# ma921/BASQ

Measured on NVIDIA B200. Metric: candidate points recombined/sec (N->n, d=10), higher is better.
Workload: dtype f32 kernel evaluation (fp16 hi/lo split distance contraction, 3 products), f64 accumulation/projection/Caratheodory

## Files before the change

basq_b200/_lib.py:

```python
from __future__ import annotations

import ctypes as C
import os

_HERE = os.path.dirname(os.path.abspath(__file__))
LIB_PATH = os.environ.get("BASQ_B200_LIB") or os.path.join(_HERE, "libbasq_b200.so")

BASQ_MAX_DIM = 32
OK, ERR_INVALID, ERR_CUDA, ERR_NUMERIC, ERR_UNSUPPORTED = range(5)
RBF, MATERN15, MATERN25 = 0, 1, 2
PLAIN, PRED_COV, WSABI_L, WSABI_M, MMLT_G = 0, 1, 2, 3, 4
F32, F64 = 0, 1
PHASES = ("prepare", "set_sum", "projection", "caratheodory", "apply", "nystrom", "gp_predict", "other")


class BasqError(RuntimeError):
    def __init__(self, code, msg):
        super().__init__(f"basq_b200 error {code}: {msg}")
        self.code = code


class KernelDesc(C.Structure):
    _fields_ = [
        ("family", C.c_int32), ("mode", C.c_int32), ("dtype", C.c_int32), ("d", C.c_int32),
# ... 33 lines not shown
        "basq_nystrom_basis_sharded": (I, [P, KD, P, L, I, P, I, I, I, P, P, P, P, P]),
        "basq_nystrom_basis": (I, [P, KD, P, L, I, P, I, P, P]),
        "basq_features": (I, [P, KD, P, L, P, L, P, I, P]),
        "basq_car": (I, [P, P, I, I, I, P, C.POINTER(I)]),
        "basq_recombine": (I, [P, KD, P, L, P, L, P, I, P, P, P, C.POINTER(I)]),
        "basq_recombine_objective": (I, [P, KD, P, L, P, L, P, I, P, P, P, P, C.POINTER(I)]),
        "basq_car_objective": (I, [P, P, I, I, I, P]),
        "basq_session_set_objective": (I, [P, P]),
        "basq_recombine_host": (I, [P, KD, P, L, P, L, P, I, P, I, P, P, P, C.POINTER(I)]),
        "basq_session_create": (I, [P, KD, P, L, L, L, P, L, P, I, P, C.POINTER(P)]),
        "basq_session_destroy": (None, [P]),
        "basq_session_count": (I, [P, C.POINTER(L)]),
        "basq_session_partial": (I, [P, L, L, P]),
        "basq_session_apply": (I, [P, L, L, P, C.POINTER(L)]),
        "basq_session_result": (I, [P, P, P, I, C.POINTER(I)]),
        "basq_session_cell_factor": (I, [P, L, L, C.POINTER(I)]),
        "basq_session_pass_begin": (I, [P, L, L, I]),
        "basq_session_level": (I, [P, I, I, P, P, P, P]),
        "basq_session_landmarks": (I, [P, C.POINTER(I)]),
        "basq_session_level_fold": (I, [P, I, I, P, P, L]),
        "basq_session_level_project": (I, [P, I, I, P, P, P, P, L, I, I, P]),
        "basq_session_apply_cells": (I, [P, L, L, I, P, C.POINTER(L)]),
        "basq_sample_mvn": (I, [P, C.c_uint64, L, L, I, I, P, P, P]),
        "basq_standard_normals": (I, [P, C.c_uint64, L, L, I, P]),
        "basq_ctx_set_seed": (I, [P, C.c_uint64]),
        "basq_ctx_memory": (I, [P, C.POINTER(C.c_uint64), C.POINTER(C.c_uint64), C.POINTER(L)]),
        "basq_ctx_allow_f32_eval": (I, [P, I, C.POINTER(L)]),
        "basq_mvn_logpdf": (I, [P, P, L, I, I, P, P, P]),
        "basq_candidate_weights": (I, [P, I, D, I, P, P, L, I, P]),
        "basq_cleanse_weights": (I, [P, P, L, D]),
        "basq_sir_resample": (I, [P, P, L, L, C.c_uint64, P, C.POINTER(L)]),
        "basq_dgemm": (I, [P, I, I, I, I, I, D, P, I, P, I, D, P, I]),
        "basq_tgemm": (I, [P, I, I, I, P, I, P, I, P, I]),
    }
    for name, (res, args) in sig.items():
        fn = getattr(lib, name)
        fn.restype = res
        fn.argtypes = args
    return lib, tuple(sig)


lib, SYMBOLS = _load()


def check(code):
    if code != OK:
        raise BasqError(code, lib.basq_last_error().decode("utf-8", "replace"))


class Context:

    def __init__(self, device_index: int, stream_ptr: int = 0):
        h = C.c_void_p()
        check(lib.basq_ctx_create(int(device_index), C.c_void_p(stream_ptr or None), C.byref(h)))
        self.handle = h
        self.device_index = device_index
        self.stream_ptr = stream_ptr

    def __del__(self):
        h, self.handle = getattr(self, "handle", None), None
        if h and lib is not None:
            lib.basq_ctx_destroy(h)

    @property
    def launches(self) -> int:
        return int(lib.basq_ctx_launch_count(self.handle))
# ... 55 lines not shown
```

basq_b200/csrc/api.cu:

```cuda
#include <math.h>
#include <string.h>
#include <stdlib.h>

#include <algorithm>
#include <memory>
#include <new>

#include "common.cuh"
#include "tgemm.cuh"

namespace basq {
const char* last_error_cstr();

namespace {

__global__ void scale_columns_kernel(double* __restrict__ U, int rows, int cols, int64_t ld,
                                     const double* __restrict__ s) {
  const int64_t t = (int64_t)blockIdx.x * blockDim.x + threadIdx.x;
  if (t >= (int64_t)rows * cols) return;
  const int r = (int)(t / cols), c = (int)(t % cols);
  U[(int64_t)r * ld + c] *= s[c];
}

__global__ void warp_gram_kernel(double* __restrict__ C, int64_t a, int64_t b, int mode, const double* __restrict__ fx,
                                 const double* __restrict__ fy, double pre_add, double diag_add, int64_t diag_col0) {
  const int64_t t = (int64_t)blockIdx.x * blockDim.x + threadIdx.x;
  if (t >= a * b) return;
  const int64_t i = t / b, j = t % b - diag_col0;
  double c = C[t];
  if (i == j) c += pre_add;
  if (mode == BASQ_WSABI_L) c = fx[i] * c * fy[j + diag_col0];
  else if (mode == BASQ_WSABI_M) c = fx[i] * c * fy[j + diag_col0] + 0.5 * c * c;
  else if (mode == BASQ_MMLT_G) c = fx[i] * fy[j + diag_col0] * expm1(c);
  if (i == j) c += diag_add;
  C[t] = c;
}

__global__ void model_space_kernel(int mode, double offset, int64_t n, double* __restrict__ mean,
                                   double* __restrict__ var, int write_var) {
  const int64_t p = (int64_t)blockIdx.x * blockDim.x + threadIdx.x;
  if (p >= n) return;
// ... 63 lines not shown

int narrow_f64(basq_ctx* ctx, const double* in, int64_t n, float* out) {
  f64_to_f32_kernel<<<(unsigned)ceil_div64(n, 256), 256, 0, ctx->stream>>>(in, n, out);
  ctx->launches++;
  BASQ_CUDA(cudaGetLastError());
  return BASQ_OK;
}

int widen_f32(basq_ctx* ctx, const float* in, int64_t n, double* out) {
  f32_to_f64_kernel<<<(unsigned)ceil_div64(n, 256), 256, 0, ctx->stream>>>(in, n, out);
  ctx->launches++;
  BASQ_CUDA(cudaGetLastError());
  return BASQ_OK;
}

namespace {

int check_finite_host(const double* v, int64_t n, const char* what) {
  for (int64_t i = 0; i < n; ++i)
    BASQ_CHECK(isfinite(v[i]), BASQ_ERR_NUMERIC, "%s contains a non-finite value at %lld", what, (long long)i);
  return BASQ_OK;
}

}
}

using namespace basq;

struct Piece {
  void* p = nullptr;
  template <typename T> T* as() const { return static_cast<T*>(p); }
};

struct basq_session {
  basq_ctx* ctx = nullptr;
  basq_kernel_desc desc;
  KParams kp;
  int M = 0, q = 0, n = 0, S = 0, Mtot = 0;
  int nl = NL_LIN;
  Landmarks lm;
  Landmarks lmobs;
  DevBuf Uprime;
  DevBuf sz;
  DevBuf Az;
  RecPool pool;
  DevBuf G;
  int64_t ldg = 0;
  DevBuf rank;
  int pass_F = 0;
  int64_t pass_R = 0, pass_off = 0;
  const double* obj = nullptr;
  int rows = 0;
  DevBuf cellmass;
  DevBuf cellobj;
  DevBuf Gf;
  DevBuf raw[2];
  int raw_cur = 0;
  DevBuf lnode, lppos, lfpar;
  NlSweep nls;
  DevBuf X64, Z64, Xobs64;
  bool promoted = false;
  double kappa = 0.0;
  int64_t idx_base = 0;
  bool scale_wf = true;
  std::vector<double> omega_host;
  std::vector<int> rank_host;
  DevBuf X32, Z32, Xobs32;
  bool demoted = false;
  const void *origX = nullptr, *origZ = nullptr, *origXobs = nullptr;
};

namespace basq {
namespace {

int session_set_sums(basq_session* s, int64_t off, int S, int64_t p_lo, int64_t p_hi, double* G, int64_t ldg) {
// ... 172 lines not shown
      s->Az.release();
      basq_kernel_desc d64 = *desc;
      d64.dtype = BASQ_F64;
      d64.Xobs = s->Xobs64.p;
      s->promoted = true;
      ctx->promotions++;
      return session_create_impl(ctx, &d64, s->X64.p, N_loc, N_glob, idx_base, s->Z64.p, M, U, q, mu, S_override, s);
    }
  }

  DevBuf sx;
  const bool has_factor = (mode == BASQ_WSABI_L || mode == BASQ_WSABI_M || mode == BASQ_MMLT_G);
  if (has_factor) {
    BASQ_TRY(s->sz.alloc(ctx, sizeof(double) * M));
    BASQ_TRY(warp_factor(ctx, desc, s->kp, s->lmobs.view(), Z, M, s->sz.as<double>()));
    BASQ_TRY(sx.alloc(ctx, sizeof(double) * std::max<int64_t>(N_loc, 1)));
    BASQ_TRY(warp_factor(ctx, desc, s->kp, s->lmobs.view(), X, N_loc, sx.as<double>()));
  }

  BASQ_TRY(s->Uprime.alloc(ctx, sizeof(double) * (size_t)q * s->Mtot));
  BASQ_CUDA(cudaMemcpy2DAsync(s->Uprime.p, sizeof(double) * s->Mtot, U, sizeof(double) * M, sizeof(double) * M, q,
                              cudaMemcpyDeviceToDevice, ctx->stream));
  if (mode == BASQ_WSABI_L) {
    scale_columns_kernel<<<ceil_div((int64_t)q * M, 256), 256, 0, ctx->stream>>>(s->Uprime.as<double>(), q, (int)M,
                                                                                s->Mtot, s->sz.as<double>());
    ctx->launches++;
  }
  if (augment) {
    BASQ_TRY(dgemm(ctx, false, false, q, n_obs, (int)M, -1.0, s->Uprime.as<double>(), s->Mtot, s->Az.as<double>(),
                   n_obs, 0.0, s->Uprime.as<double>() + M, s->Mtot));
    BASQ_CUDA(cudaStreamSynchronize(ctx->stream));
    s->Az.release();
  }

  const double uniform_w = 1.0 / (double)(N_glob > 0 ? N_glob : 1);
  BASQ_TRY(build_records(ctx, s->kp, desc->dtype, X, N_loc, uniform_w, mu, has_factor ? sx.as<double>() : nullptr,
                         !nonlin, &s->pool));

  s->ldg = 0;
  if (nonlin) {
    BASQ_TRY(nl_sweep_prepare(ctx, desc, s->kp, s->Az.as<double>(), (int)M, s->sz.as<double>(), N_loc, &s->nls));
    if (s->nls.use_nls) s->Az.release();
  }
  BASQ_CUDA(cudaStreamSynchronize(ctx->stream));
  return BASQ_OK;
}

int session_reserve_cells(basq_session* s, int cells) {
  if (cells <= s->ldg) return BASQ_OK;
  basq_ctx* ctx = s->ctx;
  BASQ_CUDA(cudaStreamSynchronize(ctx->stream));
  s->G.release();
  s->rank.release();
  s->ldg = cells;
  BASQ_TRY(s->G.alloc(ctx, sizeof(double) * (size_t)s->Mtot * s->ldg));
  BASQ_TRY(s->rank.alloc(ctx, sizeof(int) * (size_t)cells));
  s->cellmass.release();
  s->cellobj.release();
  BASQ_TRY(s->cellmass.alloc(ctx, sizeof(double) * (size_t)cells));
  BASQ_TRY(s->cellobj.alloc(ctx, sizeof(double) * (size_t)cells));
  s->omega_host.resize(cells);
  s->rank_host.resize(cells);
  return BASQ_OK;
}

int session_pass_begin(basq_session* s, int64_t R_glob, int64_t off, int F) {
// ... 83 lines not shown
  const int n = s->n, S = s->S, F = s->pass_F, rows = s->rows;
  BASQ_TRY(session_level_check(s, lvl, K, node_host, ppos_host));
  BASQ_CHECK(row0 >= 0 && nrows >= 0 && row0 + nrows <= s->Mtot, BASQ_ERR_INVALID, "level: bad landmark row range");
  const int stride = S << lvl, cnt = F >> lvl;
  PhaseTimer t(ctx, PH_PROJ);
  {
    unsigned char* slot = nullptr;
    int si = 0;
    BASQ_TRY(stage_take(ctx, (size_t)s->S * 16, &slot, &si));
    int* h_node = reinterpret_cast<int*>(slot);
    int* h_ppos = h_node + S;
    double* h_fpar = reinterpret_cast<double*>(slot + (size_t)S * 8);
    memcpy(h_node, node_host, sizeof(int) * K);
    if (lvl > 0) memcpy(h_ppos, ppos_host, sizeof(int) * K);
    memcpy(h_fpar, fpar_host, sizeof(double) * K);
    BASQ_CUDA(cudaMemcpyAsync(s->lnode.p, h_node, sizeof(int) * K, cudaMemcpyHostToDevice, ctx->stream));
    if (lvl > 0) BASQ_CUDA(cudaMemcpyAsync(s->lppos.p, h_ppos, sizeof(int) * K, cudaMemcpyHostToDevice, ctx->stream));
    BASQ_CUDA(cudaMemcpyAsync(s->lfpar.p, h_fpar, sizeof(double) * K, cudaMemcpyHostToDevice, ctx->stream));
    BASQ_CUDA(cudaEventRecord(ctx->stage_ev[si], ctx->stream));
  }
  BASQ_CUDA(cudaMemsetAsync(A_out, 0, sizeof(double) * (size_t)rows * S, ctx->stream));
  double* raw = s->raw[s->raw_cur].as<double>();
  const double* prev = s->raw[s->raw_cur ^ 1].as<double>();
  fold_cols_kernel<<<(unsigned)ceil_div64(K, 256), 256, 0, ctx->stream>>>(s->cellmass.as<double>(), 0, 1, K,
                                                                          s->lnode.as<int>(), stride, cnt, raw, S);
  ctx->launches++;
  BASQ_CUDA(cudaGetLastError());
  if (s->obj) {
    fold_cols_kernel<<<(unsigned)ceil_div64(K, 256), 256, 0, ctx->stream>>>(s->cellobj.as<double>(), 0, 1, K,
                                                                            s->lnode.as<int>(), stride, cnt,
                                                                            raw + (int64_t)n * S, S);
    ctx->launches++;
  }
  if (nrows > 0) {
    BASQ_TRY(dgemm(ctx, false, false, s->q, K, nrows, 1.0, s->Uprime.as<double>() + row0, s->Mtot, Gf_rows, ld_gf, 0.0,
                   raw + S, S));
  } else {
    BASQ_CUDA(cudaMemset2DAsync(raw + S, sizeof(double) * S, 0, sizeof(double) * K, s->q, ctx->stream));
  }
  level_finish_kernel<<<(unsigned)ceil_div64((int64_t)rows * K, 256), 256, 0, ctx->stream>>>(
      raw, prev, rows, K, lvl > 0 ? 1 : 0, s->lppos.as<int>(), s->lfpar.as<double>(), A_out, S);
  ctx->launches++;
  BASQ_CUDA(cudaGetLastError());
  s->raw_cur ^= 1;
  return BASQ_OK;
}

int session_level(basq_session* s, int lvl, int K, const int* node_host, const int* ppos_host,
                  const double* fpar_host, double* A_out) {
  const int cnt = s->pass_F >> lvl;
  bool identity = (cnt == 1 && lvl == 0);
  for (int i = 0; identity && i < K; ++i) identity = node_host[i] == i;
  if (identity)
    return session_level_project(s, lvl, K, node_host, ppos_host, fpar_host, s->G.as<double>(), s->ldg, 0, s->Mtot, A_out);
  BASQ_TRY(session_level_fold(s, lvl, K, node_host, s->Gf.as<double>(), s->S));
  return session_level_project(s, lvl, K, node_host, ppos_host, fpar_host, s->Gf.as<double>(), s->S, 0, s->Mtot, A_out);
}

struct LevelTree {
  int S = 0, F = 1, L = 0, lvl = 0;
  std::vector<int> act;
  std::vector<double> fac;
  std::vector<int> node, ppos;
  std::vector<double> fpar;
  void begin(int S_, int F_, int64_t R_glob) {
    S = S_; F = F_; lvl = 0; L = 0;
    while ((1 << L) < F) ++L;
// ... 365 lines not shown

int basq_ctx_profile_read(basq_ctx* ctx, double* ms_host, int64_t* calls_host, int reset) {
  BASQ_CHECK(ctx && ms_host, BASQ_ERR_INVALID, "NULL argument");
  ctx->resolve_spans();
  for (int i = 0; i < PH_COUNT; ++i) {
    ms_host[i] = ctx->phase_ms[i];
    if (calls_host) calls_host[i] = ctx->phase_calls[i];
    if (reset) {
      ctx->phase_ms[i] = 0.0;
      ctx->phase_calls[i] = 0;
    }
  }
  return BASQ_OK;
}

int basq_dgemm(basq_ctx* ctx, int transA, int transB, int m, int n, int k, double alpha, const double* A, int lda,
               const double* B, int ldb, double beta, double* C, int ldc) {
  BASQ_CHECK(ctx && A && B && C, BASQ_ERR_INVALID, "basq_dgemm: NULL argument");
  BASQ_CUDA(cudaSetDevice(ctx->device));
  return dgemm(ctx, transA != 0, transB != 0, m, n, k, alpha, A, lda, B, ldb, beta, C, ldc);
}

int basq_tgemm(basq_ctx* ctx, int m, int n, int k, const double* A, int lda, const double* B, int ldb, double* C,
               int ldc) {
  BASQ_CHECK(ctx && A && B && C, BASQ_ERR_INVALID, "basq_tgemm: NULL argument");
  BASQ_CHECK(m >= 1 && n >= 1 && k >= 1 && lda >= k && ldb >= k && ldc >= n, BASQ_ERR_INVALID, "basq_tgemm: bad shape");
  BASQ_CUDA(cudaSetDevice(ctx->device));
  BlkOperand a, b;
  BASQ_TRY(a.alloc(ctx, m, k));
  BASQ_TRY(b.alloc(ctx, n, k));
  BASQ_TRY(blk_from_f64(ctx, A, lda, false, &a));
  BASQ_TRY(blk_from_f64(ctx, B, ldb, false, &b));
  BASQ_TRY(tgemm(ctx, a, b, 1.0, C, ldc, false));
  BASQ_CUDA(cudaStreamSynchronize(ctx->stream));
  return BASQ_OK;
}

int basq_gram(basq_ctx* ctx, const basq_kernel_desc* desc, const void* X, int64_t a, const void* Y, int64_t b,
              double* out) {
  BASQ_CHECK(ctx && desc && X && Y && out, BASQ_ERR_INVALID, "basq_gram: NULL argument");
  BASQ_CHECK(a >= 1 && b >= 1, BASQ_ERR_INVALID, "basq_gram: empty operand");
  BASQ_CUDA(cudaSetDevice(ctx->device));
  const int rc = basq::gram_matrix(ctx, desc, X, a, Y, b, out, false);
  basq_ctx_trim(ctx, -1);
  return rc;
}

}

int basq::gram_matrix(basq_ctx* ctx, const basq_kernel_desc* desc, const void* X, int64_t a, const void* Y, int64_t b,
                      double* out, bool tensor_correction, int64_t diag_col0) {
  KParams kp;
  BASQ_TRY(make_kparams(desc, &kp));
  BASQ_TRY(compute_center(ctx, desc, X, a, &kp));
  Landmarks lmx;
  BASQ_TRY(prep_landmarks(ctx, kp, desc->dtype, X, a, nullptr, 0, &lmx));
  BASQ_TRY(base_gram(ctx, kp, lmx.view(), Y, b, out, b));
  const int mode = desc->mode;
  if (mode != BASQ_PLAIN) {
    const int n_obs = desc->n_obs;
    Landmarks lmobs;
    BASQ_TRY(prep_landmarks(ctx, kp, desc->dtype, desc->Xobs, n_obs, nullptr, 0, &lmobs));
    DevBuf KxX, T, KXy, fx, fy;
    BASQ_TRY(KxX.alloc(ctx, sizeof(double) * (size_t)a * n_obs));
    BASQ_TRY(T.alloc(ctx, sizeof(double) * (size_t)a * n_obs));
    BASQ_TRY(KXy.alloc(ctx, sizeof(double) * (size_t)n_obs * b));
// ... 441 lines not shown
```

basq_b200/csrc/setsum_mma.cuh:

```cuda
#pragma once
#include <cuda_fp16.h>

#include "common.cuh"

namespace basq {

struct SetSumMmaDev {
  const unsigned char* recs;
  int64_t count;
  int64_t off;
  int S;
  int64_t p_lo, p_hi;
  const float* lmA;
  int Mtot;
  int n_mgroups;
  int n_jgroups;
  float os_f;
  double* G;
  int64_t ldg;
  int accumulate;
};

template <int DP>
struct MmaCfg {
// ... 56 lines not shown
__device__ __forceinline__ void bulk_g2s(void* dst, const void* src, uint32_t bytes, uint64_t* bar) {
  asm volatile("cp.async.bulk.shared::cluster.global.mbarrier::complete_tx::bytes [%0], [%1], %2, [%3];" ::"r"(
                   smem_u32(dst)),
               "l"(src), "r"(bytes), "r"(smem_u32(bar))
               : "memory");
}
__device__ __forceinline__ void fence_proxy_async() { asm volatile("fence.proxy.async.shared::cta;" ::: "memory"); }
__device__ __forceinline__ void fence_barrier_init() { asm volatile("fence.mbarrier_init.release.cluster;" ::: "memory"); }
__device__ __forceinline__ void tc_fence_before() { asm volatile("tcgen05.fence::before_thread_sync;" ::: "memory"); }
__device__ __forceinline__ void tc_fence_after() { asm volatile("tcgen05.fence::after_thread_sync;" ::: "memory"); }
__device__ __forceinline__ void tmem_alloc(uint32_t* dst_smem, uint32_t cols) {
  asm volatile("tcgen05.alloc.cta_group::1.sync.aligned.shared::cta.b32 [%0], %1;" ::"r"(smem_u32(dst_smem)), "r"(cols)
               : "memory");
  asm volatile("tcgen05.relinquish_alloc_permit.cta_group::1.sync.aligned;" ::: "memory");
}
__device__ __forceinline__ void tmem_dealloc(uint32_t addr, uint32_t cols) {
  asm volatile("tcgen05.dealloc.cta_group::1.sync.aligned.b32 %0, %1;" ::"r"(addr), "r"(cols) : "memory");
}
__device__ __forceinline__ void umma_commit(uint64_t* bar) {
  asm volatile("tcgen05.commit.cta_group::1.mbarrier::arrive::one.shared::cluster.b64 [%0];" ::"r"(smem_u32(bar))
               : "memory");
}
__device__ __forceinline__ void umma_f16(uint32_t d_tmem, uint64_t adesc, uint64_t bdesc, uint32_t idesc,
                                         uint32_t accumulate) {
  asm volatile(
      "{\n"
      ".reg .pred p;\n"
      "setp.ne.b32 p, %4, 0;\n"
      "tcgen05.mma.cta_group::1.kind::f16 [%0], %1, %2, %3, p;\n"
      "}" ::"r"(d_tmem),
      "l"(adesc), "l"(bdesc), "r"(idesc), "r"(accumulate)
      : "memory");
}
__device__ __forceinline__ uint64_t smem_desc(uint32_t saddr, uint32_t lbo_bytes, uint32_t sbo_bytes) {
  uint64_t d = 0;
  d |= (uint64_t)((saddr & 0x3FFFFu) >> 4);
  d |= (uint64_t)(lbo_bytes >> 4) << 16;
  d |= (uint64_t)(sbo_bytes >> 4) << 32;
  d |= (uint64_t)1 << 46;
  return d;
}
__device__ __forceinline__ void tmem_ld32(uint32_t taddr, uint32_t (&v)[32]) {
  asm volatile(
      "tcgen05.ld.sync.aligned.32x32b.x32.b32 "
      "{%0, %1, %2, %3, %4, %5, %6, %7, %8, %9, %10, %11, %12, %13, %14, %15, "
      "%16, %17, %18, %19, %20, %21, %22, %23, %24, %25, %26, %27, %28, %29, %30, %31}, [%32];"
      : "=r"(v[0]), "=r"(v[1]), "=r"(v[2]), "=r"(v[3]), "=r"(v[4]), "=r"(v[5]), "=r"(v[6]), "=r"(v[7]), "=r"(v[8]),
        "=r"(v[9]), "=r"(v[10]), "=r"(v[11]), "=r"(v[12]), "=r"(v[13]), "=r"(v[14]), "=r"(v[15]), "=r"(v[16]),
        "=r"(v[17]), "=r"(v[18]), "=r"(v[19]), "=r"(v[20]), "=r"(v[21]), "=r"(v[22]), "=r"(v[23]), "=r"(v[24]),
        "=r"(v[25]), "=r"(v[26]), "=r"(v[27]), "=r"(v[28]), "=r"(v[29]), "=r"(v[30]), "=r"(v[31])
      : "r"(taddr)
      : "memory");
}
__device__ __forceinline__ void tmem_ld16x256_x4(uint32_t taddr, uint32_t (&v)[16]) {
  asm volatile(
      "tcgen05.ld.sync.aligned.16x256b.x4.b32 "
      "{%0, %1, %2, %3, %4, %5, %6, %7, %8, %9, %10, %11, %12, %13, %14, %15}, [%16];"
      : "=r"(v[0]), "=r"(v[1]), "=r"(v[2]), "=r"(v[3]), "=r"(v[4]), "=r"(v[5]), "=r"(v[6]), "=r"(v[7]), "=r"(v[8]),
        "=r"(v[9]), "=r"(v[10]), "=r"(v[11]), "=r"(v[12]), "=r"(v[13]), "=r"(v[14]), "=r"(v[15])
      : "r"(taddr)
      : "memory");
}
__device__ __forceinline__ void tmem_ld_wait() { asm volatile("tcgen05.wait::ld.sync.aligned;" ::: "memory"); }
__device__ __forceinline__ void named_bar_sync(int id, int nthreads) {
  asm volatile("bar.sync %0, %1;" ::"r"(id), "r"(nthreads) : "memory");
}
// ... 426 lines not shown
```

basq_b200/ops.py:

```python
from __future__ import annotations

import ctypes as C

import numpy as np
import torch

from . import _lib
from .kernels import KernelSpec, describe_kernel


def _prep(x: torch.Tensor, device, dtype):
    return x.detach().to(device=device, dtype=dtype).contiguous()


def _common(kernel, X, device=None):
    spec = describe_kernel(kernel)
    device = torch.device(device) if device is not None else X.device
    dtype = X.dtype if X.dtype in (torch.float32, torch.float64) else torch.float32
    ctx = _lib.context_for(device)
    return spec, ctx, device, dtype


def gram(kernel, X, Y, device=None) -> torch.Tensor:
    spec, ctx, device, dtype = _common(kernel, X, device)
# ... 80 lines not shown
    return Phi


def caratheodory(A: torch.Tensor) -> torch.Tensor:
    ctx = _lib.context_for(A.device)
    Ad = A.detach().to(torch.float64).contiguous().clone()
    n, S = Ad.shape
    omega = torch.zeros(S, dtype=torch.float64, device=A.device)
    _lib.check(_lib.lib.basq_car(ctx.handle, Ad.data_ptr(), n, S, S, omega.data_ptr(), None))
    return omega


def dgemm(A, B, transA=False, transB=False):
    ctx = _lib.context_for(A.device)
    A = A.contiguous(); B = B.contiguous()
    m = A.shape[1] if transA else A.shape[0]
    k = A.shape[0] if transA else A.shape[1]
    n = B.shape[0] if transB else B.shape[1]
    Cm = torch.empty(m, n, dtype=torch.float64, device=A.device)
    _lib.check(_lib.lib.basq_dgemm(ctx.handle, int(transA), int(transB), m, n, k, 1.0, A.data_ptr(), A.shape[1],
                                   B.data_ptr(), B.shape[1], 0.0, Cm.data_ptr(), n))
    return Cm


def tgemm(A, B):
    ctx = _lib.context_for(A.device)
    A = A.to(torch.float64).contiguous(); B = B.to(torch.float64).contiguous()
    m, k = A.shape
    n = B.shape[0]
    assert B.shape[1] == k
    Cm = torch.empty(m, n, dtype=torch.float64, device=A.device)
    _lib.check(_lib.lib.basq_tgemm(ctx.handle, m, n, k, A.data_ptr(), k, B.data_ptr(), k, Cm.data_ptr(), n))
    return Cm


def recombine(kernel, pts_rec, pts_nys, U, mu=None, device=None, obj=None):
    spec, ctx, device, dtype = _common(kernel, pts_rec, device)
    Xd, Zd = _prep(pts_rec, device, dtype), _prep(pts_nys, device, dtype)
    Ud = _prep(U, device, torch.float64)
    q = Ud.shape[0]
    if Ud.shape[1] != len(Zd):
        raise ValueError(f"U has {Ud.shape[1]} columns for {len(Zd)} Nystrom points")
    mud = None
    if mu is not None:
        mud = _prep(mu, device, torch.float64)
        if mud.shape != (len(Xd),):
            raise ValueError("init_weights must have one entry per candidate")
    desc, keep = spec.to_desc(Xd.shape[1], device, dtype)
    idx = torch.empty(q + 1, dtype=torch.int64, device=device)
    w = torch.empty(q + 1, dtype=torch.float64, device=device)
    n_out = C.c_int(0)
    if obj is not None:
        objd = _prep(obj, device, torch.float64)
        if objd.shape != (len(Xd),):
            raise ValueError("obj must have one entry per candidate")
        _lib.check(_lib.lib.basq_recombine_objective(ctx.handle, C.byref(desc), Xd.data_ptr(), len(Xd), Zd.data_ptr(),
                                                     len(Zd), Ud.data_ptr(), q,
                                                     mud.data_ptr() if mud is not None else None, objd.data_ptr(),
                                                     idx.data_ptr(), w.data_ptr(), C.byref(n_out)))
        return idx[: n_out.value], w[: n_out.value]
    _lib.check(_lib.lib.basq_recombine(ctx.handle, C.byref(desc), Xd.data_ptr(), len(Xd), Zd.data_ptr(), len(Zd),
                                       Ud.data_ptr(), q, mud.data_ptr() if mud is not None else None,
                                       idx.data_ptr(), w.data_ptr(), C.byref(n_out)))
    return idx[: n_out.value], w[: n_out.value]


# ... 201 lines not shown
```

include/basq_b200.h:

```cpp
#ifndef BASQ_B200_H
#define BASQ_B200_H

#include <stdint.h>

#ifdef __cplusplus
extern "C" {
#endif

#define BASQ_ABI_VERSION 2
#define BASQ_MAX_DIM 32
#define BASQ_MAX_CELL_FACTOR 16

enum basq_status {
  BASQ_OK = 0,
  BASQ_ERR_INVALID = 1,
  BASQ_ERR_CUDA = 2,
  BASQ_ERR_NUMERIC = 3,
  BASQ_ERR_UNSUPPORTED = 4
};

enum basq_family { BASQ_RBF = 0, BASQ_MATERN15 = 1, BASQ_MATERN25 = 2 };

enum basq_mode {
  BASQ_PLAIN = 0,
// ... 93 lines not shown
int basq_session_apply(basq_session* s, int64_t R_glob, int64_t off_glob, const double* omega,
                       int64_t* R_loc_new_host);
int basq_session_result(basq_session* s, int64_t* idx_out, double* w_out, int cap, int* n_out_host);

int basq_session_cell_factor(const basq_session* s, int64_t R_glob, int64_t R_loc_max, int* F_out_host);
int basq_session_pass_begin(basq_session* s, int64_t R_glob, int64_t off_glob, int F);
int basq_session_level(basq_session* s, int lvl, int K, const int* node_host, const int* ppos_host,
                       const double* fpar_host, double* A_out);
int basq_session_landmarks(const basq_session* s, int* Mtot_out_host);
int basq_session_level_fold(basq_session* s, int lvl, int K, const int* node_host, double* Gf_out, int64_t ld_gf);
int basq_session_level_project(basq_session* s, int lvl, int K, const int* node_host, const int* ppos_host,
                               const double* fpar_host, const double* Gf_rows, int64_t ld_gf, int row0,
                               int nrows, double* A_out);
int basq_session_apply_cells(basq_session* s, int64_t R_glob, int64_t off_glob, int F,
                             const double* factor_host, int64_t* R_loc_new_host);
int basq_sample_mvn(basq_ctx* ctx, uint64_t seed, int64_t offset, int64_t N, int d, int dtype,
                    const double* mean_host, const double* chol_host, void* X_out);
int basq_standard_normals(basq_ctx* ctx, uint64_t seed, int64_t offset, int64_t rows, int cols, double* out);
int basq_mvn_logpdf(basq_ctx* ctx, const void* X, int64_t N, int d, int dtype, const double* mean_host,
                    const double* chol_host, double* out);
int basq_candidate_weights(basq_ctx* ctx, int kind, double ratio, int log_out, const double* mean,
                           const double* var, int64_t N, int normalise, double* w_out);
int basq_cleanse_weights(basq_ctx* ctx, double* w, int64_t N, double eps);

int basq_sir_resample(basq_ctx* ctx, const double* w, int64_t N, int64_t n_out, uint64_t seed,
                      int64_t* idx_out_host, int64_t* n_drawn_host);

int basq_dgemm(basq_ctx* ctx, int transA, int transB, int m, int n, int k, double alpha,
               const double* A, int lda, const double* B, int ldb, double beta, double* C, int ldc);

int basq_tgemm(basq_ctx* ctx, int m, int n, int k, const double* A, int lda, const double* B, int ldb,
               double* C, int ldc);

#ifdef __cplusplus
}
#endif
#endif
```

Before: 81.77 million.

## Emulate f64 projection GEMM with int8 digit-split tcgen05 tensor-core MMA

Adds an Ozaki-style int8 GEMM: f64 operands get per-row exponents and are split into 8 signed 7-bit digits, multiplied with tcgen05 kind::i8 MMAs into TMEM diagonal accumulators, and recombined in f64. The level projection in sessions uses it in place of dgemm when q>=512 and Mtot>=8192. The aim is to replace slow FP64 GEMM throughput with int8 tensor-core throughput, at the cost of extra digit-splitting passes per call. It also risks small accuracy differences from the per-row scaling.

```diff
diff --git a/basq_b200/_lib.py b/basq_b200/_lib.py
--- a/basq_b200/_lib.py
+++ b/basq_b200/_lib.py
@@ -89,6 +89,7 @@
         "basq_sir_resample": (I, [P, P, L, L, C.c_uint64, P, C.POINTER(L)]),
         "basq_dgemm": (I, [P, I, I, I, I, I, D, P, I, P, I, D, P, I]),
         "basq_tgemm": (I, [P, I, I, I, P, I, P, I, P, I]),
+        "basq_igemm": (I, [P, I, I, I, P, I, I, I, P, I, P, I, I]),
     }
     for name, (res, args) in sig.items():
         fn = getattr(lib, name)
diff --git a/basq_b200/csrc/api.cu b/basq_b200/csrc/api.cu
--- a/basq_b200/csrc/api.cu
+++ b/basq_b200/csrc/api.cu
@@ -7,6 +7,7 @@
 #include <new>
 
 #include "common.cuh"
+#include "igemm.cuh"
 #include "tgemm.cuh"
 
 namespace basq {
@@ -136,6 +137,8 @@
   template <typename T> T* as() const { return static_cast<T*>(p); }
 };
 
+constexpr int INT8_PROJ_MIN_Q = 512, INT8_PROJ_MIN_MTOT = 8192;
+
 struct basq_session {
   basq_ctx* ctx = nullptr;
   basq_kernel_desc desc;
@@ -145,6 +148,8 @@
   Landmarks lm;
   Landmarks lmobs;
   DevBuf Uprime;
+  bool int8_proj = false;
+  DigOperand Udig, Gdig;
   DevBuf sz;
   DevBuf Az;
   RecPool pool;
@@ -383,6 +388,8 @@
     BASQ_CUDA(cudaStreamSynchronize(ctx->stream));
     s->Az.release();
   }
+  s->int8_proj = q >= INT8_PROJ_MIN_Q && s->Mtot >= INT8_PROJ_MIN_MTOT;
+  if (s->int8_proj) BASQ_TRY(dig_from_f64(ctx, s->Uprime.as<double>(), s->Mtot, false, q, s->Mtot, 0, 128, &s->Udig));
 
   const double uniform_w = 1.0 / (double)(N_glob > 0 ? N_glob : 1);
   BASQ_TRY(build_records(ctx, s->kp, desc->dtype, X, N_loc, uniform_w, mu, has_factor ? sx.as<double>() : nullptr,
@@ -532,7 +539,10 @@
                                                                             raw + (int64_t)n * S, S);
     ctx->launches++;
   }
-  if (nrows > 0) {
+  if (nrows > 0 && s->int8_proj) {
+    BASQ_TRY(dig_from_f64(ctx, Gf_rows, ld_gf, true, K, nrows, row0, 64, &s->Gdig));
+    BASQ_TRY(igemm(ctx, s->Udig, s->Gdig, 1.0, raw + S, S, false));
+  } else if (nrows > 0) {
     BASQ_TRY(dgemm(ctx, false, false, s->q, K, nrows, 1.0, s->Uprime.as<double>() + row0, s->Mtot, Gf_rows, ld_gf, 0.0,
                    raw + S, S));
   } else {
@@ -964,6 +974,21 @@
   BASQ_TRY(blk_from_f64(ctx, A, lda, false, &a));
   BASQ_TRY(blk_from_f64(ctx, B, ldb, false, &b));
   BASQ_TRY(tgemm(ctx, a, b, 1.0, C, ldc, false));
+  BASQ_CUDA(cudaStreamSynchronize(ctx->stream));
+  return BASQ_OK;
+}
+
+int basq_igemm(basq_ctx* ctx, int m, int n, int k, const double* A, int lda, int row0, int nrows, const double* B,
+               int ldb, double* C, int ldc, int accumulate) {
+  BASQ_CHECK(ctx && A && B && C, BASQ_ERR_INVALID, "basq_igemm: NULL argument");
+  BASQ_CHECK(m >= 1 && n >= 1 && k >= 1 && lda >= k && row0 >= 0 && nrows >= 1 && row0 + nrows <= k && ldb >= n &&
+                 ldc >= n,
+             BASQ_ERR_INVALID, "basq_igemm: bad shape");
+  BASQ_CUDA(cudaSetDevice(ctx->device));
+  DigOperand a, b;
+  BASQ_TRY(dig_from_f64(ctx, A, lda, false, m, k, 0, 128, &a));
+  BASQ_TRY(dig_from_f64(ctx, B, ldb, true, n, nrows, row0, 64, &b));
+  BASQ_TRY(igemm(ctx, a, b, 1.0, C, ldc, accumulate != 0));
   BASQ_CUDA(cudaStreamSynchronize(ctx->stream));
   return BASQ_OK;
 }
diff --git a/basq_b200/csrc/igemm.cu b/basq_b200/csrc/igemm.cu
--- /dev/null
+++ b/basq_b200/csrc/igemm.cu
@@ -0,0 +1,305 @@
+#include <math_constants.h>
+
+#include <algorithm>
+
+#include "common.cuh"
+#include "igemm.cuh"
+#include "setsum_mma.cuh"
+
+namespace basq {
+
+namespace {
+
+constexpr int IG_BM = 128, IG_BN = 64;
+constexpr int IG_NDIAG = IG_DIGITS;
+constexpr int IG_A_BYTES = IG_DIGITS * IG_KB * IG_BM;
+constexpr int IG_B_BYTES = IG_DIGITS * IG_KB * IG_BN;
+constexpr int IG_STAGE_BYTES = IG_A_BYTES + IG_B_BYTES;
+constexpr int IG_NSTAGE = 4;
+constexpr int IG_SMEM = IG_NSTAGE * IG_STAGE_BYTES + 256;
+constexpr int IG_THREADS = 192;
+constexpr int IG_KMAX_BLOCKS = 2047;
+static_assert(IG_NDIAG * IG_BN <= 512, "the diagonal accumulators must fit the 512 TMEM columns");
+static_assert((IG_DIGITS) * IG_KMAX_BLOCKS * (int64_t)IG_KB * 4096 < (int64_t(1) << 31), "s32 diagonal sum overflows");
+
+struct IgDev {
+  const int8_t *A, *B;
+  const int *ea, *eb;
+  int I, J;
+  int KB_A, KB_B;
+  int a_kb, b_kb;
+  int nkb;
+  double* out;
+  int64_t ldo;
+  double alpha;
+  int accumulate;
+};
+
+__global__ void __launch_bounds__(IG_THREADS, 1) igemm_kernel(const IgDev a) {
+  extern __shared__ __align__(1024) unsigned char smem_ig[];
+  unsigned char* const smem = smem_ig;
+  uint64_t* bars = reinterpret_cast<uint64_t*>(smem + IG_NSTAGE * IG_STAGE_BYTES);
+  uint64_t* s_full = bars;
+  uint64_t* s_empty = bars + IG_NSTAGE;
+  uint64_t* t_full = bars + 2 * IG_NSTAGE;
+  uint32_t* tmem_slot = reinterpret_cast<uint32_t*>(t_full + 1);
+
+  const int tid = threadIdx.x, warp = tid >> 5, lane = tid & 31;
+  const int tb = blockIdx.x, ta = blockIdx.y;
+  if (tid == 0) {
+    for (int s = 0; s < IG_NSTAGE; ++s) {
+      mma::mbar_init(&s_full[s], 1);
+      mma::mbar_init(&s_empty[s], 1);
+    }
+    mma::mbar_init(t_full, 1);
+    mma::fence_barrier_init();
+  }
+  if (warp == 1) mma::tmem_alloc(tmem_slot, 512);
+  mma::tc_fence_before();
+  __syncthreads();
+  mma::tc_fence_after();
+  const uint32_t tmem_base = *tmem_slot;
+
+  if (warp == 0) {
+    if (lane == 0) {
+      const int8_t* pa = a.A + ((size_t)ta * a.KB_A + a.a_kb) * IG_A_BYTES;
+      const int8_t* pb = a.B + ((size_t)tb * a.KB_B + a.b_kb) * IG_B_BYTES;
+      for (int kb = 0; kb < a.nkb; ++kb) {
+        const int s = kb % IG_NSTAGE;
+        mma::mbar_wait(&s_empty[s], ((kb / IG_NSTAGE) & 1u) ^ 1u);
+        unsigned char* st = smem + (size_t)s * IG_STAGE_BYTES;
+        mma::mbar_expect_tx(&s_full[s], IG_STAGE_BYTES);
+        mma::bulk_g2s(st, pa + (size_t)kb * IG_A_BYTES, IG_A_BYTES, &s_full[s]);
+        mma::bulk_g2s(st + IG_A_BYTES, pb + (size_t)kb * IG_B_BYTES, IG_B_BYTES, &s_full[s]);
+      }
+    }
+  } else if (warp == 1) {
+    constexpr uint32_t IDESC = (2u << 4) | (1u << 7) | (1u << 10) | ((uint32_t)(IG_BM >> 4) << 24);
+    for (int kb = 0; kb < a.nkb; ++kb) {
+      const int s = kb % IG_NSTAGE;
+      mma::mbar_wait(&s_full[s], (kb / IG_NSTAGE) & 1u);
+      mma::tc_fence_after();
+      if (lane == 0) {
+        const uint32_t st = mma::smem_u32(smem + (size_t)s * IG_STAGE_BYTES);
+#pragma unroll
+        for (int da = 0; da < IG_DIGITS; ++da) {
+          const uint64_t ad = mma::smem_desc(st + da * (IG_BM * 16), IG_DIGITS * IG_BM * 16, 128);
+#pragma unroll
+          for (int db = 0; db < IG_DIGITS - da; db += 4) {
+            const int n = min(4, IG_DIGITS - da - db) * IG_BN;
+            const uint64_t bd = mma::smem_desc(st + IG_A_BYTES + db * (IG_BN * 16), IG_DIGITS * IG_BN * 16, 128);
+            mma::umma_i8(tmem_base + (uint32_t)((da + db) * IG_BN), ad, bd, IDESC | ((uint32_t)(n >> 3) << 17),
+                         (kb > 0 || da > 0) ? 1u : 0u);
+          }
+        }
+        mma::umma_commit(&s_empty[s]);
+        if (kb == a.nkb - 1) mma::umma_commit(t_full);
+      }
+      __syncwarp();
+    }
+  } else {
+    const int quarter = warp & 3;
+    const int i = ta * IG_BM + quarter * 32 + lane;
+    mma::mbar_wait(t_full, 0);
+    mma::tc_fence_after();
+    const uint32_t taddr = tmem_base + ((uint32_t)(quarter * 32) << 16);
+    const int ea = (i < a.I) ? a.ea[i] : 0;
+#pragma unroll 1
+    for (int cb = 0; cb < IG_BN; cb += 32) {
+      double acc[32];
+#pragma unroll
+      for (int c = 0; c < 32; ++c) acc[c] = 0.0;
+#pragma unroll 1
+      for (int t = IG_NDIAG - 1; t >= 0; --t) {
+        uint32_t v[32];
+        mma::tmem_ld32(taddr + (uint32_t)(t * IG_BN + cb), v);
+        mma::tmem_ld_wait();
+#pragma unroll
+        for (int c = 0; c < 32; ++c) acc[c] = acc[c] * 0.0078125 + (double)(int)v[c];
+      }
+      if (i < a.I) {
+        const int j0 = tb * IG_BN + cb;
+#pragma unroll
+        for (int c = 0; c < 32; ++c) {
+          const int j = j0 + c;
+          if (j >= a.J) continue;
+          const int eb = a.eb[j];
+          const double val = (ea == IG_NONFINITE || eb == IG_NONFINITE) ? CUDART_NAN : a.alpha * ldexp(acc[c], ea + eb);
+          double* dst = a.out + (int64_t)i * a.ldo + j;
+          *dst = a.accumulate ? *dst + val : val;
+        }
+      }
+    }
+  }
+
+  mma::tc_fence_before();
+  __syncthreads();
+  if (warp == 1) {
+    mma::tc_fence_after();
+    mma::tmem_dealloc(tmem_base, 512);
+  }
+}
+
+__global__ void ig_rowmax_kernel(const double* __restrict__ src, int64_t ld, int kdim,
+                                 unsigned long long* __restrict__ mx_bits) {
+  __shared__ double sh[256];
+  const int row = blockIdx.x;
+  double mx = 0.0;
+  for (int k = threadIdx.x; k < kdim; k += 256) {
+    const double v = fabs(src[(int64_t)row * ld + k]);
+    mx = (v == v) ? fmax(mx, v) : CUDART_INF;
+  }
+  sh[threadIdx.x] = mx;
+  __syncthreads();
+  for (int w = 128; w > 0; w >>= 1) {
+    if ((int)threadIdx.x < w) sh[threadIdx.x] = fmax(sh[threadIdx.x], sh[threadIdx.x + w]);
+    __syncthreads();
+  }
+  if (threadIdx.x == 0) mx_bits[row] = (unsigned long long)__double_as_longlong(sh[0]);
+}
+
+__global__ void ig_rowmax_t_kernel(const double* __restrict__ src, int64_t ld, int rows, int kdim, int kslice,
+                                   unsigned long long* __restrict__ mx_bits) {
+  __shared__ double sh[8][33];
+  const int tx = threadIdx.x & 31, ty = threadIdx.x >> 5;
+  const int row = blockIdx.x * 32 + tx;
+  const int k0 = blockIdx.y * kslice, k1 = min(kdim, k0 + kslice);
+  double mx = 0.0;
+  if (row < rows)
+    for (int k = k0 + ty; k < k1; k += 8) {
+      const double v = fabs(src[(int64_t)k * ld + row]);
+      mx = (v == v) ? fmax(mx, v) : CUDART_INF;
+    }
+  sh[ty][tx] = mx;
+  __syncthreads();
+  if (ty == 0 && row < rows) {
+    for (int y = 1; y < 8; ++y) mx = fmax(mx, sh[y][tx]);
+    atomicMax(&mx_bits[row], (unsigned long long)__double_as_longlong(mx));
+  }
+}
+
+__global__ void ig_rowexp_kernel(const unsigned long long* __restrict__ mx_bits, int rows, int padded,
+                                 int* __restrict__ rexp) {
+  const int row = blockIdx.x * blockDim.x + threadIdx.x;
+  if (row >= padded) return;
+  int e = 0;
+  if (row < rows) {
+    const double mx = __longlong_as_double((long long)mx_bits[row]);
+    if (!isfinite(mx)) {
+      e = IG_NONFINITE;
+    } else if (mx > 0.0) {
+      frexp(mx, &e);
+      e -= 6;
+    }
+  }
+  rexp[row] = e;
+}
+
+template <bool TRANSPOSED>
+__global__ void ig_split_kernel(const double* __restrict__ src, int64_t ld, int rows, int kdim, int k0, int kb0, int RT,
+                                int KB, int tile, const int* __restrict__ rexp, int8_t* __restrict__ dig) {
+  const int64_t t = (int64_t)blockIdx.x * blockDim.x + threadIdx.x;
+  if (t >= (int64_t)RT * KB * 2 * tile) return;
+  const int r = (int)(t % tile);
+  const int h = (int)((t / tile) & 1);
+  const int kb = (int)((t / (2 * tile)) % KB);
+  const int rt = (int)(t / (2 * (int64_t)tile * KB));
+  const int row = rt * tile + r;
+  const int e = rexp[row];
+  const int kfirst = (kb0 + kb) * IG_KB + h * 16 - k0;
+  uint32_t w[IG_DIGITS][4];
+#pragma unroll
+  for (int da = 0; da < IG_DIGITS; ++da)
+#pragma unroll
+    for (int q = 0; q < 4; ++q) w[da][q] = 0u;
+#pragma unroll
+  for (int u = 0; u < 16; ++u) {
+    const int k = kfirst + u;
+    double y = 0.0;
+    if (row < rows && k >= 0 && k < kdim && e != IG_NONFINITE)
+      y = ldexp(TRANSPOSED ? src[(int64_t)k * ld + row] : src[(int64_t)row * ld + k], -e);
+#pragma unroll
+    for (int da = 0; da < IG_DIGITS; ++da) {
+      const double d = rint(y);
+      w[da][u >> 2] |= ((uint32_t)(int)d & 0xFFu) << (8 * (u & 3));
+      y = (y - d) * 128.0;
+    }
+  }
+  int8_t* base = dig + (((size_t)rt * KB + kb) * 2 + h) * IG_DIGITS * tile * 16 + (size_t)r * 16;
+#pragma unroll
+  for (int da = 0; da < IG_DIGITS; ++da)
+    *reinterpret_cast<uint4*>(base + (size_t)da * tile * 16) = make_uint4(w[da][0], w[da][1], w[da][2], w[da][3]);
+}
+
+}
+
+int dig_from_f64(basq_ctx* ctx, const double* src, int64_t ld, bool transposed, int rows, int kdim, int k0, int tile,
+                 DigOperand* op) {
+  BASQ_CHECK(rows >= 0 && kdim >= 1 && k0 >= 0 && (tile == IG_BM || tile == IG_BN), BASQ_ERR_INVALID,
+             "dig_from_f64: bad shape (rows %d, kdim %d, k0 %d, tile %d)", rows, kdim, k0, tile);
+  op->rows = rows;
+  op->tile = tile;
+  op->RT = std::max(1, ceil_div(rows, tile));
+  op->kb0 = k0 / IG_KB;
+  op->KB = ceil_div((int64_t)k0 + kdim, IG_KB) - op->kb0;
+  const int padded = op->RT * tile;
+  BASQ_TRY(op->dig.alloc(ctx, (size_t)op->RT * op->KB * IG_DIGITS * IG_KB * tile));
+  BASQ_TRY(op->rexp.alloc(ctx, sizeof(int) * (size_t)padded));
+  DevBuf mx;
+  BASQ_TRY(mx.alloc(ctx, sizeof(unsigned long long) * (size_t)padded));
+  if (rows > 0) {
+    if (transposed) {
+      BASQ_CUDA(cudaMemsetAsync(mx.p, 0, sizeof(unsigned long long) * (size_t)rows, ctx->stream));
+      const int slices = std::max(1, std::min(64, kdim / 128));
+      const int kslice = ceil_div(kdim, slices);
+      ig_rowmax_t_kernel<<<dim3((unsigned)ceil_div(rows, 32), (unsigned)ceil_div(kdim, kslice)), 256, 0, ctx->stream>>>(
+          src, ld, rows, kdim, kslice, mx.as<unsigned long long>());
+    } else {
+      ig_rowmax_kernel<<<rows, 256, 0, ctx->stream>>>(src, ld, kdim, mx.as<unsigned long long>());
+    }
+    ctx->launches++;
+  }
+  ig_rowexp_kernel<<<ceil_div(padded, 256), 256, 0, ctx->stream>>>(mx.as<unsigned long long>(), rows, padded,
+                                                                   op->rexp.as<int>());
+  const int64_t total = (int64_t)op->RT * op->KB * 2 * tile;
+  const unsigned grid = (unsigned)ceil_div64(total, 256);
+  if (transposed)
+    ig_split_kernel<true><<<grid, 256, 0, ctx->stream>>>(src, ld, rows, kdim, k0, op->kb0, op->RT, op->KB, tile,
+                                                         op->rexp.as<int>(), op->dig.as<int8_t>());
+  else
+    ig_split_kernel<false><<<grid, 256, 0, ctx->stream>>>(src, ld, rows, kdim, k0, op->kb0, op->RT, op->KB, tile,
+                                                          op->rexp.as<int>(), op->dig.as<int8_t>());
+  ctx->launches += 2;
+  BASQ_CUDA(cudaGetLastError());
+  return BASQ_OK;
+}
+
+int igemm(basq_ctx* ctx, const DigOperand& A, const DigOperand& B, double alpha, double* out, int64_t ldo,
+          bool accumulate) {
+  BASQ_CHECK(A.tile == IG_BM && B.tile == IG_BN, BASQ_ERR_INVALID, "igemm: operand tiles %d / %d (need %d / %d)", A.tile,
+             B.tile, IG_BM, IG_BN);
+  BASQ_CHECK(B.kb0 >= A.kb0 && B.kb0 + B.KB <= A.kb0 + A.KB, BASQ_ERR_INVALID,
+             "igemm: K blocks [%d, %d) of B lie outside A's [%d, %d)", B.kb0, B.kb0 + B.KB, A.kb0, A.kb0 + A.KB);
+  BASQ_CHECK((size_t)IG_SMEM <= ctx->smem_optin, BASQ_ERR_UNSUPPORTED, "igemm: needs %d B shared memory", IG_SMEM);
+  if (A.rows <= 0 || B.rows <= 0) return BASQ_OK;
+  IgDev d;
+  d.A = A.dig.as<int8_t>(); d.B = B.dig.as<int8_t>();
+  d.ea = A.rexp.as<int>(); d.eb = B.rexp.as<int>();
+  d.I = A.rows; d.J = B.rows;
+  d.KB_A = A.KB; d.KB_B = B.KB;
+  d.out = out; d.ldo = ldo;
+  d.alpha = alpha;
+  BASQ_CUDA(cudaFuncSetAttribute(igemm_kernel, cudaFuncAttributeMaxDynamicSharedMemorySize, IG_SMEM));
+  for (int kb = 0; kb < B.KB; kb += IG_KMAX_BLOCKS) {
+    d.b_kb = kb;
+    d.a_kb = B.kb0 - A.kb0 + kb;
+    d.nkb = std::min(IG_KMAX_BLOCKS, B.KB - kb);
+    d.accumulate = (accumulate || kb > 0) ? 1 : 0;
+    igemm_kernel<<<dim3((unsigned)B.RT, (unsigned)A.RT), IG_THREADS, IG_SMEM, ctx->stream>>>(d);
+    ctx->launches++;
+    BASQ_CUDA(cudaGetLastError());
+  }
+  return BASQ_OK;
+}
+
+}
diff --git a/basq_b200/csrc/igemm.cuh b/basq_b200/csrc/igemm.cuh
--- /dev/null
+++ b/basq_b200/csrc/igemm.cuh
@@ -0,0 +1,23 @@
+#pragma once
+#include "common.cuh"
+
+namespace basq {
+
+constexpr int IG_DIGITS = 8;
+constexpr int IG_KB = 32;
+
+struct DigOperand {
+  DevBuf dig;
+  DevBuf rexp;
+  int rows = 0, tile = 0, RT = 0;
+  int kb0 = 0, KB = 0;
+};
+constexpr int IG_NONFINITE = 1 << 30;
+
+int dig_from_f64(basq_ctx* ctx, const double* src, int64_t ld, bool transposed, int rows, int kdim, int k0, int tile,
+                 DigOperand* op);
+
+int igemm(basq_ctx* ctx, const DigOperand& A, const DigOperand& B, double alpha, double* out, int64_t ldo,
+          bool accumulate);
+
+}
diff --git a/basq_b200/csrc/setsum_mma.cuh b/basq_b200/csrc/setsum_mma.cuh
--- a/basq_b200/csrc/setsum_mma.cuh
+++ b/basq_b200/csrc/setsum_mma.cuh
@@ -112,6 +112,17 @@
       "l"(adesc), "l"(bdesc), "r"(idesc), "r"(accumulate)
       : "memory");
 }
+__device__ __forceinline__ void umma_i8(uint32_t d_tmem, uint64_t adesc, uint64_t bdesc, uint32_t idesc,
+                                        uint32_t accumulate) {
+  asm volatile(
+      "{\n"
+      ".reg .pred p;\n"
+      "setp.ne.b32 p, %4, 0;\n"
+      "tcgen05.mma.cta_group::1.kind::i8 [%0], %1, %2, %3, p;\n"
+      "}" ::"r"(d_tmem),
+      "l"(adesc), "l"(bdesc), "r"(idesc), "r"(accumulate)
+      : "memory");
+}
 __device__ __forceinline__ uint64_t smem_desc(uint32_t saddr, uint32_t lbo_bytes, uint32_t sbo_bytes) {
   uint64_t d = 0;
   d |= (uint64_t)((saddr & 0x3FFFFu) >> 4);
diff --git a/basq_b200/ops.py b/basq_b200/ops.py
--- a/basq_b200/ops.py
+++ b/basq_b200/ops.py
@@ -136,6 +136,22 @@
     Cm = torch.empty(m, n, dtype=torch.float64, device=A.device)
     _lib.check(_lib.lib.basq_tgemm(ctx.handle, m, n, k, A.data_ptr(), k, B.data_ptr(), k, Cm.data_ptr(), n))
     return Cm
+
+
+def igemm(A, B, row0=0, out=None):
+    ctx = _lib.context_for(A.device)
+    A = A.to(torch.float64).contiguous(); B = B.to(torch.float64).contiguous()
+    m, k = A.shape
+    nrows, n = B.shape
+    if row0 < 0 or row0 + nrows > k:
+        raise ValueError(f"rows [{row0}, {row0 + nrows}) of B lie outside A's {k} columns")
+    accumulate = out is not None
+    if out is None:
+        out = torch.empty(m, n, dtype=torch.float64, device=A.device)
+    assert out.shape == (m, n) and out.dtype == torch.float64 and out.is_contiguous()
+    _lib.check(_lib.lib.basq_igemm(ctx.handle, m, n, k, A.data_ptr(), k, row0, nrows, B.data_ptr(), n,
+                                   out.data_ptr(), n, int(accumulate)))
+    return out
 
 
 def recombine(kernel, pts_rec, pts_nys, U, mu=None, device=None, obj=None):
diff --git a/include/basq_b200.h b/include/basq_b200.h
--- a/include/basq_b200.h
+++ b/include/basq_b200.h
@@ -149,6 +149,9 @@
 int basq_tgemm(basq_ctx* ctx, int m, int n, int k, const double* A, int lda, const double* B, int ldb,
                double* C, int ldc);
 
+int basq_igemm(basq_ctx* ctx, int m, int n, int k, const double* A, int lda, int row0, int nrows, const double* B,
+               int ldb, double* C, int ldc, int accumulate);
+
 #ifdef __cplusplus
 }
 #endif
```

New measurement: 88.73 million, median of 6. 8.5% higher.
